# siyarvurucu/gym-macm

Measured on AMD Instinct MI355X. Metric: agent·steps/sec, cm-flock-v0 64 agents × 4096 envs, at 1/2/4/8 MI355X, higher is better.
Workload: dtype f32; 1 GPU; cm-flock-v0 n_agents=[64] x 4096 envs per GPU, uniform random discrete actions (MultiDiscrete[3,3,3]) pre-generated on device, from reset (seed 0x6d61636d); envs_per_gpu=4096, n_agents=64, total_envs=4096, split=weak: 4096 envs per GPU, parallelism=env-sharded x1 (no data-path collective), obs=float32, max_contacts=2016, spill_slots=4096, launch=one macm_world_rollout_traj launch for the K timed steps, outputs=every step's ([K, E, N, ...] trajectory buffers)

## Files before the change

### gym-macm_amd/csrc/flock_step_w64.hip

```cpp
#include "bots.hpp"
#include "flock_common.hpp"
#include "flock_spill.hpp"
#include "tdm_obs.hpp"

namespace macm {

constexpr int W = 64;
constexpr int TCAP = 256;
constexpr int DEG = 16;
constexpr int ICAP = W / 2;
constexpr int RCH = 2;
constexpr int KREC = 4;
constexpr int KRECA = KREC;
constexpr int kLevelsMinIsland = 4;
constexpr int kPrio2T = 3;

#if defined(MACM_STAMPS) && !defined(MACM_TIMELINE)
#define STAMP(k)                                                                    \
  do {                                                                              \
    __builtin_amdgcn_s_waitcnt(0);                                                  \
    const unsigned long long _t = __builtin_amdgcn_s_memtime();                     \
    if (lane == 0) B.stamps[(size_t)e * 16 + (k)] = _t;                             \
  } while (0)
#define STAMP_STAT(k, v)                                                            \
// ... 495 lines not shown
    win[2 * (K % kNearAhead)] = s_pc2[K + kNearAhead];
    win[2 * (K % kNearAhead) + 1] = s_pc2[16 + K + kNearAhead];
  }
  near2_min<2 * K, 32 + 2 * K, SCAL>(qa.x, qa.y, qb.x, qb.y, cme, st);
  near2_min<2 * K + 1, 33 + 2 * K, SCAL>(qa.z, qa.w, qb.z, qb.w, cme, st);
  if constexpr ((K & 1) == 1) __builtin_amdgcn_sched_barrier(0);
  if constexpr (K + 1 < 16) near2_step<K + 1, SCAL>(s_pc2, win, cme, st);
}

__device__ __forceinline__ unsigned long long moved_pairs(unsigned long long movedm, float4 fn, int lane) {
  unsigned long long row = 0ull;
  for (unsigned long long m = movedm; m; m &= m - 1ull) {
    const int j = __builtin_ctzll(m);
    const float jx = bcast(fn.x, j), jy = bcast(fn.y, j), jz = bcast(fn.z, j), jw = bcast(fn.w, j);
    const float sepv = fmaxf(fmaxf(jx - fn.z, jy - fn.w), fmaxf(fn.x - jz, fn.y - jw));
    const bool ov = !(0.0f < sepv);
    const unsigned long long colj = __ballot(ov);
    row |= (ov ? (1ull << j) : 0ull) | (lane == j ? colj : 0ull);
  }
  return row;
}

__device__ __forceinline__ int write_new_pairs(int lane, unsigned long long newmask, uint32_t* ocab,
                                               float2* ocimp, int C) {
  const int cnt = __popcll(newmask);
  const int pre = wave_prefix_sum(cnt);
  const int total = __builtin_amdgcn_readlane(pre, W - 1);
  int w = total - pre;
  unsigned long long m = newmask;
  while (m) {
    const int j = 63 - __clzll(m);
    m &= ~(1ull << j);
    if (w < C) {
      st_g<kState>(ocab + w, (uint32_t)lane | ((uint32_t)j << 16));
      st_g<kState>(ocimp + w, make_float2(0.0f, 0.0f));
    }
    ++w;
  }
  return total;
}

struct TailObs {
  unsigned long long* ctl;
  unsigned int tag;
  int nsteps;
  int k;
  bool worker;
  bool more;
  int q, left;
  int r, r_end;
  int nq;
};
constexpr int kTailChunk = 2;
constexpr unsigned kTailSpins = 1u << 20;

__device__ __forceinline__ unsigned long long* tail_counter(const TailObs& tl, int q) {
  return tl.ctl + (size_t)(((tl.tag & 1u) * kTailQ + q) * kTailLine);
}
// ... 56 lines not shown
    tl.more = false;
    return;
  }
  const size_t srow = ((size_t)k * E + e) * N;
  float4 sn = make_float4(0.0f, 0.0f, 0.0f, 0.0f);
  if (lane < N) sn = ld_wt4(TB.snap_out + srow + lane);
  const size_t row = ((size_t)(tl.k + k) * E + e) * N;
  s_c[lane] = make_float2(sn.x, sn.y);
  s_ang[lane] = sn.z;
  const unsigned long long livem = __ballot(lane < N && sn.w != 0.0f);
  __syncthreads();
  const size_t slots = row * (N - 1);
  OT* const obs_r = obs ? obs + slots * 4 : nullptr;
  uint8_t* const mask_r = TB.mask_out ? TB.mask_out + slots : nullptr;
  if constexpr (sizeof(OT) == 4) {
    if (staged) tdm_obs_rowblocks<OT>(obs_r, mask_r, N, lane, livem, TP, s_c, s_ang, stage, true);
    else tdm_obs_pairs<OT>(obs_r, mask_r, N, lane, livem, TP, s_c, s_ang);
  } else {
    tdm_obs_pairs<OT>(obs_r, mask_r, N, lane, livem, TP, s_c, s_ang);
  }
  __syncthreads();
}

template <int MODE, int NCAP, typename OT, bool SCAL = false>
__device__ __attribute__((always_inline)) inline void step_w64_body(
    const StepParams& P, const WorldBuffers& B, const TdmParams& TP, const TdmBuffers& TB, int cur,
    const void* __restrict__ actions, OT* __restrict__ obs, int32_t* __restrict__ nbr_out,
    float* __restrict__ rew_out, uint8_t* __restrict__ coll_out, uint8_t* __restrict__ done_out,
    const int e = blockIdx.x, const int lane = threadIdx.x, TailObs* tl = nullptr) {
  constexpr bool kT = MODE == kTdm;
#ifdef MACM_TIMELINE
  const unsigned long long tl_rt0 = __builtin_amdgcn_s_memrealtime(), tl_c0 = __builtin_amdgcn_s_memtime();
#endif
  const int N = P.n_agents;
  const int C = P.max_contacts;
  bool act = lane < N;
  const size_t ag = (size_t)e * N + lane;
  const int nxt = cur ^ 1;
  const unsigned long long lt = lanemask_lt(lane);

  __shared__ float2 s_c[W];
  __shared__ float2 s_v[W];
  constexpr int TMW = kT ? 1 : 2;
  struct __align__(32) Pool {
    float tn[2 * TCAP];
    uint32_t tab[TCAP];
    float tln[TCAP], tlt[TCAP];
    uint32_t tm[2 * TMW * W];
    uint32_t oldm[2 * W];
  };
  __shared__ Pool s_pool;
  static_assert(spill::layout(W, !kT).total <= (int)sizeof(Pool), "the spill step must fit the pool");
  uint32_t* const s_tab = s_pool.tab;
// ... 15 lines not shown
  __shared__ uint32_t s_cvis[TCAP / 32];
  __shared__ uint8_t s_deg[W], s_stack[W], s_ibodies[W], s_bisl[W];
  __shared__ uint16_t s_ic[ICAP + 1];
  __shared__ uint8_t s_ib[ICAP + 1];
  __shared__ uint8_t s_isolved[ICAP];
  __shared__ uint32_t s_imin[ICAP];
  __shared__ int s_nisl;
  __shared__ double s_hpd[W];
  __shared__ int8_t s_hit[W];
  __shared__ float s_ang[W];
#ifdef MACM_STAMPS
  __shared__ int s_stat_maxisl;
#endif
  if constexpr (kT) {
    if (tl && tl->worker) {
      tdm_tail_row<OT>(P, B, TP, TB, obs, *tl, lane, s_c, s_ang, reinterpret_cast<float4*>(&s_pool),
                       tdm_obs_rb_stage_bytes(N) <= (int)sizeof(Pool));
      return;
    }
  }

  const uint32_t* cab = B.cab[cur] + (size_t)e * C;
  const float2* cimp = B.cimp[cur] + (size_t)e * C;
  const int step_count = B.step_count[e];
  const int M = B.ccount[cur][e];
  float2 p = make_float2(0.0f, 0.0f), v = make_float2(0.0f, 0.0f), tg = make_float2(0.0f, 0.0f);
  float ang = 0.0f, slp = 0.0f;
  float4 fo = make_float4(0.0f, 0.0f, 0.0f, 0.0f);
  int a0 = 1, a1 = 1, a2 = 1, a3 = 0;
  float ax = 0.0f, ay = 0.0f;
  double hp = 0.0, cda = 0.0, cdm = 0.0;
  if (act) {
    p = B.pos[ag];
    v = B.vel[ag];
    ang = B.angle[ag];
    fo = B.fat[ag];
    slp = B.sleep[ag];
    if constexpr (kT) {
      const uchar4 a = reinterpret_cast<const uchar4*>(actions)[ag];
      a0 = a.x;
      a1 = a.y;
      a2 = a.z;
      a3 = a.w;
      act = TB.alive[ag] != 0;
      hp = TB.health[ag];
      cda = TB.cd_atk[ag];
      cdm = TB.cd_mov[ag];
    } else if (P.action_mode == MACM_ACTION_DISCRETE) {
      const uint8_t* a = (const uint8_t*)actions + ag * 3;
      a0 = a[0];
      a1 = a[1];
      a2 = a[2];
    } else {
      const float2 c = ((const float2*)actions)[ag];
      ax = c.x;
      ay = c.y;
    }
    if constexpr (!kT) tg = B.targets[(size_t)e * P.n_targets + B.tidx[lane]];
  }
  const bool act0 = act;
  double time_passed = 0.0;
  int st_prev = 0;
  unsigned long long ctr[4] = {0ull, 0ull, 0ull, 0ull};
  int2 lis = make_int2(0, -1);
  int win_prev = -1;
  uint8_t done_prev = 0;
  if (lane == 0) {
    time_passed = B.time_passed[e];
    st_prev = B.status[e];
    if constexpr (kT) {
      lis = TB.listener[e];
      win_prev = TB.winner[e];
      done_prev = B.done[e];
    }
    const ulonglong2* ec = reinterpret_cast<const ulonglong2*>(B.env_counters + (size_t)e * 4);
    const ulonglong2 c01 = ec[0], c23 = ec[1];
    ctr[0] = c01.x;
    ctr[1] = c01.y;
    ctr[2] = c23.x;
    ctr[3] = c23.y;
  }
  uint32_t rab[RCH];
  float2 rim[RCH];
#pragma unroll
  for (int c = 0; c < RCH; ++c) {
    const int k = c * W + lane;
    rab[c] = 0u;
    rim[c] = make_float2(0.0f, 0.0f);
    if (k < M) {
      rab[c] = cab[k];
      rim[c] = cimp[k];
    }
  }
  s_c[lane] = p;
  if (lane < TCAP / 32) s_cvis[lane] = 0u;
  s_oldm[2 * lane] = 0u;
#pragma unroll
  for (int q = 0; q < 2 * TMW; ++q) s_tm[2 * TMW * lane + q] = 0u;
  s_oldm[2 * lane + 1] = 0u;
  int status = 0;
  STAMP(0);

  float Fx = 0.0f, Fy = 0.0f;
  bool attacking = false;
  float ray_x = 0.0f, ray_y = 0.0f;
  if (act) {
    if (P.action_mode == MACM_ACTION_DISCRETE) {
      float af = (float)((double)ang + ((double)(a2 - 1) * P.rot_step) * P.inv_hz);
      double ad = (double)af;
      if (fabs(ad) > M_PI) {
        af = (float)(ad - sgn(ad) * (2.0 * M_PI));
        ad = (double)af;
      }
      ang = af;
// ... 147 lines not shown
  STAMP(2);

  const bool fast_dfs = T <= 64 * TMW;
  int deg = 0;
  unsigned long long tmask = 0ull, tmask1 = 0ull;
  if (fast_dfs) {
    if (act) {
      const uint32_t* tm = s_tm + 2 * TMW * lane;
      tmask = (unsigned long long)tm[0] | ((unsigned long long)tm[1] << 32);
      if (TMW == 2 && T > 64) tmask1 = (unsigned long long)tm[2] | ((unsigned long long)tm[3] << 32);
      deg = __popcll(tmask) + __popcll(tmask1);
    }
  } else if (act) {
    for (int t = 0; t < T; ++t) {
      const uint32_t ab = s_tab[t];
      if ((int)(ab & 0xffffu) == lane || (int)(ab >> 16) == lane) {
        if (deg < DEG) s_adj[lane * DEG + deg] = (uint8_t)t;
        ++deg;
      }
    }
  }
  if constexpr (!kT) {
    if (touch_over || (!fast_dfs && __builtin_amdgcn_ballot_w64(deg > DEG) != 0ull) || P.force_spill) {
      spill::step_env<OT, true>(P, B, e, cur, actions, obs, nbr_out, rew_out, coll_out, done_out,
                                reinterpret_cast<unsigned char*>(&s_pool));
      return;
    }
  } else {
    if (touch_over || (!fast_dfs && __builtin_amdgcn_ballot_w64(deg > DEG) != 0ull) || P.force_spill) {
      __shared__ int s_slot;
      const int slot = spill::acquire_slot(B, e, &s_slot);
      if (slot < 0) {
        spill::keep_lists(P, B, e, cur);
        if (lane == 0) {
          B.status[e] |= MACM_ST_SPILL_WAIT;
          report_status(B, MACM_ST_SPILL_WAIT);
        }
        return;
      }
      if (lane < N) {
        if (act0) {
          B.angle[ag] = ang;
          TB.cd_atk[ag] = cda;
          TB.cd_mov[ag] = cdm;
        }
        TB.health[ag] = hp;
// ... 2 lines not shown
        if (TB.alive_out) TB.alive_out[ag] = act ? 1 : 0;
      }
      if (lane == 0) {
        TB.listener[e] = lis;
        ulonglong2* ec = reinterpret_cast<ulonglong2*>(B.env_counters + (size_t)e * 4);
        ec[0] = make_ulonglong2(ctr[0] + (unsigned long long)__popcll(alive0_m),
                                ctr[1] + (unsigned long long)__popcll(att_m));
        B.env_counters[(size_t)e * 4 + 2] = ctr[2] + (unsigned long long)__popcll(alive0_m & ~livem);
      }
      const float2 F1 = make_float2(Fx, Fy);
      spill::step_env<OT, false, kTdm>(P, B, e, cur, actions, obs, nullptr, nullptr, nullptr, done_out,
                                        reinterpret_cast<unsigned char*>(&s_pool), &TP, &TB, &F1, slot);
      return;
    }
  }
  if (!fast_dfs && deg > DEG) {
    status |= MACM_ST_DEGREE_OVERFLOW;
    deg = DEG;
  }
  if (!fast_dfs) s_deg[lane] = (uint8_t)deg;
  const unsigned long long hasdeg = __ballot(act && deg > 0);
  __syncthreads();
  STAMP(3);
  if (hasdeg) __builtin_amdgcn_s_setprio(3);

  uint32_t ordv = 0u, lvlv = 0u, kislv = 0u;
  bool lvl_path = fast_dfs && T <= 64;
  if (fast_dfs) {
    const uint32_t tabv = lane < T ? s_tab[lane] : 0u;
    const uint32_t tabv1 = (TMW == 2 && 64 + lane < T) ? s_tab[64 + lane] : 0u;
    const uint32_t tm_lo = (uint32_t)tmask, tm_hi = (uint32_t)(tmask >> 32);
    const uint32_t tm1_lo = (uint32_t)tmask1, tm1_hi = (uint32_t)(tmask1 >> 32);
    uint32_t ordv1 = 0u, bodv = 0u, islv = 0u, icv = 0u, ibv = 0u, stk = 0u;
    int nord = 0, nisl = 0, nb = 0;
    auto dfs = [&](auto wide) {
    constexpr bool W2 = decltype(wide)::value;
    unsigned long long vis = ~hasdeg, cvis = 0ull, cvis1 = 0ull;
    for (unsigned long long todo = hasdeg; todo; todo = hasdeg & ~vis) {
      const int s = 63 - __clzll(todo);
      icv = writelane_m0(nord, nisl, icv);
      ibv = writelane_m0(nb, nisl, ibv);
      vis |= 1ull << s;
      stk = writelane_m0(s, 0, stk);
      int sp = 1;
      while (sp > 0) {
        --sp;
// ... 563 lines not shown
      near2_step<0, SCAL>(s_pc2, win, mk2(cx, cy), s2);
      const bool upper = s2.best_b < s2.best_a;
      best = upper ? s2.best_b : s2.best_a;
      bj = upper ? s2.bj_b : s2.bj_a;
    } else {
      NearState s1;
      s1.best = best;
      s1.bj = bj;
      float4 win[kNearAhead];
#pragma unroll
      for (int k = 0; k < kNearAhead; ++k) win[k] = s_pc2[k];
      near_step<0, NCAP>(s_pc2, win, mk2(cx, cy), s1);
      best = s1.best;
      bj = s1.bj;
    }
  }
  const unsigned long long myov = moved_pairs(movedm, fn, lane) & valid & ~(1ull << lane);
  const unsigned long long oldm = (unsigned long long)s_oldm[2 * lane] | ((unsigned long long)s_oldm[2 * lane + 1] << 32);
  const bool coll = act && ((myov | oldm) != 0ull);
  const unsigned long long above = lane == 63 ? 0ull : (~0ull << (lane + 1));
  const unsigned long long newmask = act ? (myov & ~oldm & above) : 0ull;
  STAMP(10);

  uint32_t* ocab = B.cab[nxt] + (size_t)e * C;
  float2* ocimp = B.cimp[nxt] + (size_t)e * C;
  const int nnew = write_new_pairs(lane, newmask, ocab, ocimp, C);
  int kept = 0, Tr = 0;
  for (int c = 0; c * W < M; ++c) {
    const int k = c * W + lane;
    uint32_t ab = 0u;
    if (c < RCH) {
#pragma unroll
      for (int q = 0; q < RCH; ++q)
        if (q == c) ab = rab[q];
    } else if (k < M) {
      ab = cab[k];
    }
    bool keep = false;
    const bool touch = (tbits >> c) & 1u;
    if (k < M) {
      const int a = ab & 0xffffu, b = ab >> 16;
      keep = overlap(s_fn[a], s_fn[b]);
    }
    const unsigned long long mt = __ballot(touch), mk = __ballot(keep);
    const int trank = Tr + __popcll(mt & lt);
    const int krank = kept + __popcll(mk & lt);
    Tr += __popcll(mt);
    kept += __popcll(mk);
    if (keep) {
      const int w = nnew + krank;
      if (w < C) {
        float2 l = make_float2(0.0f, 0.0f);
        if (touch && trank < TCAP) l = make_float2(s_tln[trank], s_tlt[trank]);
        st_g<kState>(ocab + w, ab);
        st_g<kState>(ocimp + w, l);
      }
    }
  }
  int total = nnew + kept;
  if (total > C) {
    status |= MACM_ST_CONTACT_OVERFLOW;
    total = C;
  }
  STAMP(11);

  float rew = 0.0f;
  if constexpr (!kT) {
    if (act) {
      const float tdx = tg.x - cx, tdy = tg.y - cy;
      const float td2 = tdx * tdx + tdy * tdy;
      const double d = sqrt((double)td2);
      if (coll) rew = -1.0f;
      else if (P.reward_mode == MACM_REWARD_LINEAR) rew = (float)((-d / 35) + 1);
      else rew = (d < P.reward_radius) ? 1.0f : 0.0f;
      st_g<kOut>(rew_out + ag, rew);
      if (coll_out) st_g<kOut>(coll_out + ag, (uint8_t)(coll ? 1 : 0));
      if (nbr_out) st_g<kOut>(nbr_out + ag, (int32_t)bj);
      if (obs) {
// ... 79 lines not shown
      }
      if (alive_teams == 0) dn = 1;
      TB.winner[e] = win;
      if (TB.winner_out) TB.winner_out[e] = win;
      TB.listener[e] = lis;
    }
    B.time_passed[e] = tp;
    B.done[e] = dn;
    if (done_out) done_out[e] = dn;
    B.step_count[e] = step_count + 1;
    B.ccount[nxt][e] = total;
    const int st = (mst1 ? 1 : 0) | (mst2 ? 2 : 0) | (mst4 ? 4 : 0);
    if (st) {
      B.status[e] = st_prev | st;
      report_status(B, st);
    }
    const unsigned long long c0 = kT ? (unsigned long long)__popcll(alive0_m) : (unsigned long long)N;
    ulonglong2* ec = reinterpret_cast<ulonglong2*>(B.env_counters + (size_t)e * 4);
    ec[0] = make_ulonglong2(ctr[0] + c0, ctr[1] + c1);
    ec[1] = make_ulonglong2(ctr[2] + c2, ctr[3] + (unsigned long long)dn);
    if constexpr (!kT) {
      if (P.reward_mode == MACM_REWARD_LINEAR) add_reward_sum(B, e, rsum);
    }
  }
  STAMP(13);
#ifdef MACM_TIMELINE
  {
    const unsigned long long rt1 = __builtin_amdgcn_s_memrealtime(), c1t = __builtin_amdgcn_s_memtime();
    const unsigned long long hw = (unsigned)__builtin_amdgcn_s_getreg((31 << 11) | 4);
    const unsigned long long xcc = (unsigned)__builtin_amdgcn_s_getreg((31 << 11) | 20);
    if (lane == 0) {
      unsigned long long* st = B.stamps + (size_t)e * 16;
      st[0] = tl_rt0;
      st[1] = tl_c0;
      st[2] = hw | (xcc << 32);
      st[3] = rt1;
      st[4] = c1t;
    }
  }
#endif
  STAMP_STAT(14, (unsigned long long)T | ((unsigned long long)nisl << 16) | ((unsigned long long)M << 32));
#ifdef MACM_STAMPS
  STAMP_STAT(15, (unsigned long long)s_stat_maxisl | ((unsigned long long)total << 32));
#endif
}

// ... 1 lines not shown

template <typename OT>
struct RolloutArgs {
  StepParams P;
  WorldBuffers B;
  TdmParams TP;
  TdmBuffers TB;
  const void* actions;
  OT* obs;
  int32_t* nbr_out;
  float* rew_out;
  uint8_t* coll_out;
  uint8_t* done_out;
  unsigned long long astride;
  int cur;
  int nsteps;
  uint8_t* policy_act;
  int traj;
  int sched_off;
  unsigned long long* tail_ctl;
  unsigned int tail_tag;
  int tail_k0;
};

template <typename T>
__device__ __forceinline__ T* traj_row(T* p, size_t k, size_t per_step) {
  return p ? p + k * per_step : p;
}

constexpr int kRollBalanceMinSteps = 32;
constexpr int kSchedMaxSize = 4095;

__global__ __launch_bounds__(1024) void rollout_sched(const uint32_t* __restrict__ ccount, uint32_t* __restrict__ order,
                                                     int E, int C, unsigned int* reset2 = nullptr) {
  extern __shared__ uint32_t s_h[];
  __shared__ int s_scan[32];
  const int tid = threadIdx.x, BS = blockDim.x;
  if (reset2 && tid < 2) reset2[tid] = 0u;
  for (int i = tid; i <= C; i += BS) s_h[i] = 0u;
  __syncthreads();
  for (int e = tid; e < E; e += BS) atomicAdd(&s_h[max(0, min((int)ccount[e], C))], 1u);
  __syncthreads();
  {
    const int per = (C + 1 + BS - 1) / BS, hi = C - tid * per, lo = max(-1, hi - per);
    int sum = 0;
    for (int c = hi; c > lo; --c) sum += (int)s_h[c];
    int run;
    spill::block_scan_excl(sum, run, s_scan);
    for (int c = hi; c > lo; --c) {
      const int n = (int)s_h[c];
      s_h[c] = (uint32_t)run;
      run += n;
    }
  }
  __syncthreads();
  for (int e = tid; e < E; e += BS) order[atomicAdd(&s_h[max(0, min((int)ccount[e], C))], 1u)] = (uint32_t)e;
}

template <int MODE, int NCAP, typename OT, bool SCAL = false>
__global__ __launch_bounds__(W) __attribute__((amdgpu_waves_per_eu(4))) void env_rollout_w64(RolloutArgs<OT> A0) {
  const int nsteps = A0.nsteps;
  const bool bal = A0.B.sched && nsteps >= kRollBalanceMinSteps;
  const bool phys = MODE != kTdm || (int)blockIdx.x < A0.P.n_envs;
  const int env = bal && phys ? (int)A0.B.sched[A0.sched_off + blockIdx.x] : (int)blockIdx.x;
  const int nq = gridDim.x < (unsigned)kTailQ ? (int)gridDim.x : kTailQ;
  TailObs tl{};
  tl.ctl = A0.tail_tag ? A0.tail_ctl : nullptr;
  tl.tag = A0.tail_tag;
  tl.nsteps = nsteps - A0.tail_k0;
  tl.k = 0;
  tl.worker = false;
  tl.more = true;
  tl.q = (int)(blockIdx.x % nq);
  tl.left = 1;
  tl.r = 0;
  tl.r_end = 0;
  tl.nq = nq;
  const int ksteps = phys ? nsteps : 0;
  for (int k = 0; k < ksteps; ++k) {
    const __attribute__((address_space(4))) RolloutArgs<OT>* ka =
        (const __attribute__((address_space(4))) RolloutArgs<OT>*)__builtin_amdgcn_kernarg_segment_ptr();
    asm volatile("" : "+s"(ka));
    const RolloutArgs<OT>& A = *(const RolloutArgs<OT>*)ka;
    const int N = A.P.n_agents, lane = threadIdx.x;
    const size_t EN = (size_t)A.P.n_envs * N;
    const size_t kr = A.traj ? (size_t)k : 0;
    const size_t od = MODE == kTdm ? (size_t)(N - 1) * 4 : (A.P.coord == MACM_COORD_CARTESIAN ? 6 : 4);
    OT* const obs = traj_row(A.obs, kr, EN * od);
    TdmBuffers TB = A.TB;
    if constexpr (MODE == kTdm) {
      TB.mask_out = traj_row(TB.mask_out, kr, EN * (N - 1));
      TB.health_out = traj_row(TB.health_out, kr, EN);
      TB.alive_out = traj_row(TB.alive_out, kr, EN);
      TB.winner_out = traj_row(TB.winner_out, kr, (size_t)A.P.n_envs);
      TB.snap_out = A.tail_tag ? (k >= A.tail_k0 ? traj_row(TB.snap_out, (size_t)(k - A.tail_k0), EN) : nullptr)
                               : traj_row(TB.snap_out, kr, EN);
    }
    const size_t abytes = MODE == kTdm ? 4 : 3;
    uint8_t* const pol_in = A.policy_act ? A.policy_act + kr * EN * abytes : nullptr;
    __builtin_amdgcn_s_setprio(0);
    int sl = (int)threadIdx.x;
    if constexpr (MODE == kTdm) asm volatile("" : "+v"(sl));
    tl.k = k - A0.tail_k0;
    step_w64_body<MODE, NCAP, OT, SCAL>(A.P, A.B, A.TP, TB, A.cur ^ (k & 1),
                                        pol_in ? pol_in : static_cast<const unsigned char*>(A.actions) + (size_t)k * A.astride,
                                        obs, traj_row(A.nbr_out, kr, EN), traj_row(A.rew_out, kr, EN),
                                        traj_row(A.coll_out, kr, EN), traj_row(A.done_out, kr, (size_t)A.P.n_envs),
                                        env, sl, MODE == kTdm ? &tl : nullptr);
    __builtin_amdgcn_fence(__ATOMIC_SEQ_CST, "workgroup");
    __syncthreads();
    if (pol_in) {
      uint8_t* const pol_out = A.traj ? pol_in + EN * abytes : pol_in;
      if (lane < N) {
        const size_t row = (size_t)env * N + lane;
        if constexpr (MODE == kTdm)
          bot_combat_row(obs + row * (N - 1) * 4, TB.mask_out + row * (N - 1), N, pol_out + row * 4);
        else
          bot_flock_row(obs + row * od, (int)od, pol_out + row * 3);
      }
      __builtin_amdgcn_fence(__ATOMIC_SEQ_CST, "workgroup");
      __syncthreads();
    }
  }
  if constexpr (MODE == kTdm) {
    if (tl.ctl) {
      if (phys) {
        __builtin_amdgcn_s_waitcnt(0);
        if (threadIdx.x == 0)
          __hip_atomic_store(tl.ctl + 2 * kTailQ * kTailLine + env, ((unsigned long long)tl.tag << 32) | (unsigned)tl.nsteps,
                             __ATOMIC_RELAXED, __HIP_MEMORY_SCOPE_AGENT);
      }
      if (blockIdx.x == 0 && threadIdx.x < kTailQ)
        __hip_atomic_store(tl.ctl + (size_t)((((tl.tag + 1u) & 1u) * kTailQ + threadIdx.x) * kTailLine), 0ull,
                           __ATOMIC_RELAXED, __HIP_MEMORY_SCOPE_AGENT);
      tl.worker = true;
      tl.k = A0.tail_k0;
      int sl = (int)threadIdx.x;
      asm volatile("" : "+v"(sl));
      while (tl.more)
        step_w64_body<MODE, NCAP, OT, SCAL>(A0.P, A0.B, A0.TP, A0.TB, A0.cur, nullptr, A0.obs, nullptr, nullptr, nullptr,
                                            nullptr, env, sl, &tl);
    }
  }
}

int tdm_rollout_resident_blocks(int n_agents, bool obs_f64) {
  const void* k = n_agents <= 32 ? (obs_f64 ? (const void*)env_rollout_w64<kTdm, 32, double>
                                            : (const void*)env_rollout_w64<kTdm, 32, float>)
                                 : (obs_f64 ? (const void*)env_rollout_w64<kTdm, 64, double>
                                            : (const void*)env_rollout_w64<kTdm, 64, float>);
  int per = 0, dev = 0, cus = 0;
  if (hipOccupancyMaxActiveBlocksPerMultiprocessor(&per, k, W, 0) != hipSuccess || hipGetDevice(&dev) != hipSuccess ||
      hipDeviceGetAttribute(&cus, hipDeviceAttributeMultiprocessorCount, dev) != hipSuccess) {
    (void)hipGetLastError();
    return 0;
  }
  return per * cus;
}

template <int MODE, int NCAP, typename OT, bool SCAL = false>
static void launch_roll(int nsteps, unsigned long long astride, int traj, hipStream_t s, const StepParams& P,
                        const WorldBuffers& B, const TdmParams& TP, const TdmBuffers& TB, int cur, const void* actions,
                        void* obs, int32_t* nbr, float* rew, uint8_t* coll, uint8_t* done,
                        unsigned long long* tail_ctl = nullptr, unsigned tail_tag = 0u, int tail_workers = 0,
                        int tail_k0 = 0) {
  uint8_t* pol = astride == 0 ? static_cast<uint8_t*>(const_cast<void*>(actions)) : nullptr;
  const bool bal = B.sched && nsteps >= kRollBalanceMinSteps;
  if (bal) {
    const int CB = P.max_contacts < kSchedMaxSize ? P.max_contacts : kSchedMaxSize;
    hipLaunchKernelGGL(rollout_sched, dim3(1), dim3(1024), sizeof(uint32_t) * (CB + 1), s,
                       reinterpret_cast<const uint32_t*>(B.ccount[cur]), B.sched, P.n_envs, CB, nullptr);
    if (hipPeekAtLastError() != hipSuccess) return;
  }
  RolloutArgs<OT> A{P, B, TP, TB, actions, (OT*)obs, nbr, rew, coll, done, astride, cur, nsteps, pol, traj, 0,
                    tail_ctl, tail_tag, tail_tag ? tail_k0 : 0};
  const int blocks = P.n_envs + (tail_tag ? tail_workers : 0);
  hipLaunchKernelGGL((env_rollout_w64<MODE, NCAP, OT, SCAL>), dim3(blocks), dim3(W), 0, s, A);
}

hipError_t launch_env_order(const uint32_t* ccount, uint32_t* order, int E, int C, hipStream_t s, unsigned int* reset2) {
  const int CB = C < kSchedMaxSize ? C : kSchedMaxSize;
  hipLaunchKernelGGL(rollout_sched, dim3(1), dim3(1024), sizeof(uint32_t) * (CB + 1), s, ccount, order, E, CB, reset2);
  return hipGetLastError();
}

hipError_t launch_rollout_w64(const StepParams& P, const WorldBuffers& B, int cur, const void* actions, void* obs,
                              bool obs_f64, int32_t* nbr, float* rew, uint8_t* coll, uint8_t* done, hipStream_t s,
                              int nsteps, unsigned long long astride, int traj) {
  const TdmParams TP{};
  const TdmBuffers TB{};
  const bool small = P.n_agents <= 32;
  if (obs_f64) {
    if (small)
      launch_roll<kFlock, 32, double>(nsteps, astride, traj, s, P, B, TP, TB, cur, actions, obs, nbr, rew, coll, done);
    else
      launch_roll<kFlock, 64, double>(nsteps, astride, traj, s, P, B, TP, TB, cur, actions, obs, nbr, rew, coll, done);
  } else {
    if (small)
      launch_roll<kFlock, 32, float>(nsteps, astride, traj, s, P, B, TP, TB, cur, actions, obs, nbr, rew, coll, done);
    else if (P.n_envs >= kScalarSweepMinEnvs)
      launch_roll<kFlock, 64, float, true>(nsteps, astride, traj, s, P, B, TP, TB, cur, actions, obs, nbr, rew, coll,
                                           done);
    else
      launch_roll<kFlock, 64, float>(nsteps, astride, traj, s, P, B, TP, TB, cur, actions, obs, nbr, rew, coll, done);
  }
  return hipGetLastError();
}

hipError_t launch_tdm_rollout_w64(const StepParams& P, const WorldBuffers& B, const TdmParams& TP,
                                  const TdmBuffers& TB, int cur, const void* actions, void* obs, bool obs_f64,
                                  uint8_t* done, hipStream_t s, int nsteps, unsigned long long astride, int traj,
                                  unsigned long long* tail_ctl, unsigned tail_tag, int tail_workers,
                                  int tail_k0) {
  const bool small = P.n_agents <= 32;
  if (obs_f64) {
    if (small)
      launch_roll<kTdm, 32, double>(nsteps, astride, traj, s, P, B, TP, TB, cur, actions, obs, nullptr, nullptr,
                                    nullptr, done, tail_ctl, tail_tag, tail_workers, tail_k0);
    else
      launch_roll<kTdm, 64, double>(nsteps, astride, traj, s, P, B, TP, TB, cur, actions, obs, nullptr, nullptr,
                                    nullptr, done, tail_ctl, tail_tag, tail_workers, tail_k0);
  } else {
    if (small)
      launch_roll<kTdm, 32, float>(nsteps, astride, traj, s, P, B, TP, TB, cur, actions, obs, nullptr, nullptr,
                                   nullptr, done, tail_ctl, tail_tag, tail_workers, tail_k0);
    else
      launch_roll<kTdm, 64, float>(nsteps, astride, traj, s, P, B, TP, TB, cur, actions, obs, nullptr, nullptr,
// ... 291 lines not shown
```

### gym-macm_amd/csrc/macm_capi.hip

```cpp
#include <math.h>
#include <stdio.h>
#include <string.h>

#include <algorithm>
#include <string>
#include <vector>

#include "flock_common.hpp"
#include "py_mt19937.hpp"

namespace macm {
hipError_t launch_step_w64(const StepParams& P, const WorldBuffers& B, int cur, const void* actions, void* obs,
                           bool obs_f64, int32_t* nbr, float* rew, uint8_t* coll, uint8_t* done, hipStream_t s);
hipError_t launch_rollout_w64(const StepParams& P, const WorldBuffers& B, int cur, const void* actions, void* obs,
                              bool obs_f64, int32_t* nbr, float* rew, uint8_t* coll, uint8_t* done, hipStream_t s,
                              int nsteps, unsigned long long astride, int traj);
hipError_t launch_init_w64(const StepParams& P, const WorldBuffers& B, int cur, void* obs, bool obs_f64,
                           int32_t* nbr, const uint8_t* mask, hipStream_t s);
hipError_t launch_observe_w64(const StepParams& P, const WorldBuffers& B, void* obs, bool obs_f64, int32_t* nbr,
                              hipStream_t s);
hipError_t launch_step_wg(const StepParams& P, const WorldBuffers& B, int cur, int tcap, const void* actions,
                          void* obs, bool obs_f64, int32_t* nbr, float* rew, uint8_t* coll, uint8_t* done,
                          hipStream_t s, HandoffStream* HS, uint8_t* bot_act = nullptr);
hipError_t launch_init_wg(const StepParams& P, const WorldBuffers& B, int cur, void* obs, bool obs_f64, int32_t* nbr,
                          const uint8_t* mask, hipStream_t s);
hipError_t launch_observe_wg(const StepParams& P, const WorldBuffers& B, void* obs, bool obs_f64, int32_t* nbr,
                             hipStream_t s);
hipError_t launch_tdm_step_w64(const StepParams& P, const WorldBuffers& B, const TdmParams& TP,
                               const TdmBuffers& TB, int cur, const void* actions, void* obs, bool obs_f64,
                               uint8_t* done, hipStream_t s);
hipError_t launch_tdm_rollout_w64(const StepParams& P, const WorldBuffers& B, const TdmParams& TP,
                                  const TdmBuffers& TB, int cur, const void* actions, void* obs, bool obs_f64,
                                  uint8_t* done, hipStream_t s, int nsteps, unsigned long long astride, int traj,
                                  unsigned long long* tail_ctl = nullptr, unsigned tail_tag = 0u, int tail_workers = 0,
                                  int tail_k0 = 0);
int tdm_rollout_resident_blocks(int n_agents, bool obs_f64);
hipError_t launch_tdm_init_w64(const StepParams& P, const WorldBuffers& B, const TdmParams& TP,
                               const TdmBuffers& TB, int cur, void* obs, bool obs_f64, const uint8_t* mask,
                               hipStream_t s);
// ... 37 lines not shown

struct macm_world {
  macm_config cfg;
  StepParams P;
  WorldBuffers B;
  int cur;
  int device;
  bool wave;
  bool big;
  int tcap;
  std::vector<int32_t> tidx;
  std::vector<void*> allocs;
  uint32_t* mt = nullptr;
  uint8_t* rmask = nullptr;
  bool mt_valid = false;
  uint32_t* hstat = nullptr;
  unsigned long long* bad = nullptr;
  std::vector<hipStream_t> slice_streams;
  std::vector<hipEvent_t> slice_events;
  HandoffStream* ho = nullptr;
  bool ho_tried = false;
  int slots_alloc = 0;
  int pool0 = 0;
};

struct macm_tdm {
  macm_tdm_config cfg;
  StepParams P;
  WorldBuffers B;
  TdmParams TP;
  TdmBuffers TB;
  int cur;
  int device;
  bool wave;
  std::vector<int> team;
  std::vector<void*> allocs;
  uint32_t* mt = nullptr;
  uint8_t* rmask = nullptr;
  bool mt_valid = false;
  uint32_t* hstat = nullptr;
  unsigned long long* bad = nullptr;
  int slots_alloc = 0;
  int pool0 = 0;
  float4* snap = nullptr;
  size_t snap_rows = 0;
  hipStream_t obs_stream = nullptr;
// ... 649 lines not shown

static int world_rollout(macm_world* w, const void* actions, int n_steps, const macm_outputs* out, void* stream,
                         bool bots, bool traj) {
  if (n_steps < 0) return fail(MACM_E_INVALID, "n_steps must be >= 0");
  if (n_steps == 0) return MACM_OK;
  if (!w || !actions || !out || !out->reward) return fail(MACM_E_INVALID, "world/actions/out/reward is NULL");
  if (bots && !out->obs) return fail(MACM_E_INVALID, "out->obs is NULL (the bots act on it)");
  if (bots && w->cfg.action_mode != MACM_ACTION_DISCRETE) return fail(MACM_E_INVALID, "bots.flock acts in discrete mode");
  if (const uint32_t st = read_host_status(w->hstat)) return overflow_error(st);
  DeviceGuard g(w->device);
  hipStream_t s = (hipStream_t)stream;
  const int mode = w->cfg.action_mode == MACM_ACTION_DISCRETE ? 0 : 1;
  if (w->cfg.validate_actions) {
    const long long rows = (long long)(bots ? 1 : n_steps) * w->P.n_envs;
    if (rows > INT32_MAX) return fail(MACM_E_INVALID, "n_steps * n_envs too large to validate");
    const int rc = check_actions(w->bad, actions, mode, nullptr, (int)rows, w->P.n_agents, s, w->P.n_envs);
    if (rc) return rc;
  }
  const unsigned long long astride =
      bots ? 0ull
           : (unsigned long long)w->P.n_envs * w->P.n_agents * (mode == 0 ? 3 * sizeof(uint8_t) : 2 * sizeof(float));
  if (w->wave) {
    HIP_TRY(launch_rollout_w64(w->P, w->B, w->cur, actions, out->obs, w->cfg.obs_f64 != 0, out->nbr_id, out->reward,
                               out->collided, out->done, s, n_steps, astride, traj ? 1 : 0));
    if (n_steps & 1) w->cur ^= 1;
    return MACM_OK;
  }
  const unsigned char* act = static_cast<const unsigned char*>(actions);
  if (const int S = wg_rollout_slices(w)) return rollout_wg_slices(w, S, act, n_steps, astride, out, traj, s);
  const long long rows = (long long)w->P.n_envs * w->P.n_agents;
  const unsigned long long kstride = bots ? (traj ? (unsigned long long)rows * 3 : 0ull) : astride;
  for (int k = 0; k < n_steps; ++k) {
    const macm_outputs ok = step_outputs(w, out, k, traj);
    const unsigned char* act_k = act + k * kstride;
    if (w->big)
      HIP_TRY(launch_step_big(w->P, w->B, w->cur, act_k, ok.obs, w->cfg.obs_f64 != 0, ok.nbr_id, ok.reward,
                              ok.collided, ok.done, s));
    else
      HIP_TRY(launch_step_wg(w->P, w->B, w->cur, w->tcap, act_k, ok.obs, w->cfg.obs_f64 != 0, ok.nbr_id, ok.reward,
                             ok.collided, ok.done, s, handoff_for(w),
                             bots ? const_cast<unsigned char*>(act_k) + (traj ? rows * 3 : 0) : nullptr));
    w->cur ^= 1;
    if (bots && w->big)
      HIP_TRY(launch_bots_flock(ok.obs, w->cfg.obs_f64 != 0, obs_dim(w->cfg), rows,
                                const_cast<unsigned char*>(act_k) + (traj ? rows * 3 : 0), s));
  }
  return MACM_OK;
// ... 206 lines not shown
extern "C++" template <typename Wt>
static int set_spill_pool(Wt* w, int32_t flags, int pool) {
  const bool want = (flags & MACM_DEBUG_SPILL_POOL) != 0;
  const bool never = (flags & MACM_DEBUG_SPILL_FAIL) != 0;
  if (want && never) return fail(MACM_E_INVALID, "SPILL_POOL and SPILL_FAIL exclude each other");
  if (want && (pool < 1 || pool > w->slots_alloc))
    return fail(MACM_E_INVALID, "SPILL_POOL: 1 <= slots <= the " + std::to_string(w->slots_alloc) + " allocated");
  const int target = never ? -1 : want ? pool : w->pool0;
  if (target == w->B.sp_pool) return MACM_OK;
  DeviceGuard g(w->device);
  HIP_TRY(hipDeviceSynchronize());
  if (target > 0) {
    if (!w->B.sp_lock && dalloc(w->allocs, &w->B.sp_lock, (size_t)w->slots_alloc)) return MACM_E_OOM;
    HIP_TRY(hipMemset(w->B.sp_lock, 0, sizeof(uint32_t) * w->slots_alloc));
  }
  w->B.sp_pool = target;
  return MACM_OK;
}

int macm_world_set_debug(macm_world* w, int32_t flags) {
  if (!w) return fail(MACM_E_INVALID, "world is NULL");
  const int pool = (flags & MACM_DEBUG_SPILL_POOL) ? (flags >> 8) : 0;
  flags &= 0xff;
  if (flags & ~(MACM_DEBUG_FORCE_SPILL | MACM_DEBUG_SWEEP_CELLS | MACM_DEBUG_SWEEP_ALL_PAIRS | MACM_DEBUG_SPILL_POOL | MACM_DEBUG_SPILL_FAIL))
    return fail(MACM_E_INVALID, "unknown debug flag");
  if ((flags & MACM_DEBUG_SWEEP_CELLS) && (flags & MACM_DEBUG_SWEEP_ALL_PAIRS))
    return fail(MACM_E_INVALID, "SWEEP_CELLS and SWEEP_ALL_PAIRS exclude each other");
  if (int rc = set_spill_pool(w, flags, pool)) return rc;
  w->P.force_spill = (flags & MACM_DEBUG_FORCE_SPILL) ? 1 : 0;
  w->P.sweep = (flags & MACM_DEBUG_SWEEP_CELLS) ? 1 : (flags & MACM_DEBUG_SWEEP_ALL_PAIRS) ? 2 : 0;
  return MACM_OK;
}


int macm_tdm_config_default(macm_tdm_config* c) {
  if (!c) return fail(MACM_E_INVALID, "cfg is NULL");
  memset(c, 0, sizeof(*c));
  c->n_teams = 2;
  c->team_size[0] = 1;
  c->team_size[1] = 1;
  c->n_agents = 2;
  c->velocity_iterations = 8;
  c->position_iterations = 3;
  c->warm_starting = 1;
  c->obs_f64 = 0;
  c->fresh_raycast = 0;
  c->decay_mov_penalty = 0;
  c->hz = 60.0;
  c->world_width = 30.0;
  c->world_height = 30.0;
  c->agent_rotation_speed = 0.8 * (2 * M_PI);
  c->agent_force = 20.0;
// ... 696 lines not shown
```

### gym-macm_amd/gym_macm/_abi.py

```python
from __future__ import annotations

import ctypes
import os
from ctypes import (POINTER, Structure, c_char_p, c_double, c_float, c_int, c_int32, c_int64,
                    c_uint8, c_uint64, c_void_p)

ACTION_DISCRETE, ACTION_CONTINUOUS = 0, 1
REWARD_BINARY, REWARD_LINEAR = 0, 1
COORD_POLAR, COORD_CARTESIAN = 0, 1

ST_CONTACT_OVERFLOW, ST_TOUCH_OVERFLOW, ST_DEGREE_OVERFLOW, ST_INVALID_ACTION, ST_SPILL_WAIT = 1, 2, 4, 8, 16
ST_HANDOFF = 32
DEBUG_FORCE_SPILL = 1
DEBUG_SWEEP_CELLS = 2
DEBUG_SWEEP_ALL_PAIRS = 4
DEBUG_SPILL_POOL = 8
DEBUG_SPILL_FAIL = 16
E_INVALID, E_OVERFLOW = -1, -5

_ERRORS = {
    -1: "MACM_E_INVALID",
    -2: "MACM_E_OOM",
    -3: "MACM_E_HIP",
    -4: "MACM_E_UNSUPPORTED",
    -5: "MACM_E_OVERFLOW",
}


class MacmConfig(Structure):
    _fields_ = [
        ("n_agents", c_int32),
        ("n_targets", c_int32),
        ("action_mode", c_int32),
        ("reward_mode", c_int32),
        ("coord", c_int32),
        ("velocity_iterations", c_int32),
        ("position_iterations", c_int32),
        ("warm_starting", c_int32),
        ("obs_f64", c_int32),
        ("validate_actions", c_int32),
# ... 227 lines not shown
```

### include/macm.h

```cpp
#ifndef MACM_H
#define MACM_H

#include <stdint.h>

#ifdef __cplusplus
extern "C" {
#endif

#define MACM_ABI_VERSION 9

enum {
  MACM_OK = 0,
  MACM_E_INVALID = -1,
  MACM_E_OOM = -2,
  MACM_E_HIP = -3,
  MACM_E_UNSUPPORTED = -4,
  MACM_E_OVERFLOW = -5
};

enum { MACM_ACTION_DISCRETE = 0, MACM_ACTION_CONTINUOUS = 1 };
enum { MACM_REWARD_BINARY = 0, MACM_REWARD_LINEAR = 1 };
enum { MACM_COORD_POLAR = 0, MACM_COORD_CARTESIAN = 1 };

enum {
  MACM_ST_CONTACT_OVERFLOW = 1,
  MACM_ST_TOUCH_OVERFLOW = 2,
  MACM_ST_DEGREE_OVERFLOW = 4,
  MACM_ST_INVALID_ACTION = 8,
  MACM_ST_SPILL_WAIT = 16,
  MACM_ST_HANDOFF = 32
};

enum {
  MACM_DEBUG_FORCE_SPILL = 1,
  MACM_DEBUG_SWEEP_CELLS = 2,
  MACM_DEBUG_SWEEP_ALL_PAIRS = 4,
  MACM_DEBUG_SPILL_POOL = 8,
  MACM_DEBUG_SPILL_FAIL = 16
};

typedef struct macm_config {
  int32_t n_agents;
  int32_t n_targets;
  int32_t action_mode;
  int32_t reward_mode;
  int32_t coord;
  int32_t velocity_iterations;
  int32_t position_iterations;
  int32_t warm_starting;
  int32_t obs_f64;
  int32_t validate_actions;
  double hz;
  double start_spread;
  double start_point[2];
  double agent_rotation_speed;
  double agent_force;
  double time_limit;
  double reward_radius;
  double target_mindist;
  double target_maxdist;
  float radius;
// ... 200 lines not shown
```

Before: 22.02 billion agent·steps/s.

## Carry per-agent state and contacts in registers across rollout steps

In the Flock rollout kernel with supplied actions, each step now keeps per-agent position, velocity, angle, fatigue, sleep, target, step count, the next step's actions and up to RCH*W contact pairs and impulses in a register/LDS carry struct. The next step reads these instead of reloading them from global memory, and contacts are staged in shared memory as they are written. The aim is to cut global loads and the load latency at the start of every step. The carry is invalidated when contacts overflow, on a spill, on other status flags, or when a debug reload flag is set. The cost is more register pressure, extra LDS writes, and a more complex control path that may hurt occupancy.

```diff
diff --git a/gym-macm_amd/csrc/flock_step_w64.hip b/gym-macm_amd/csrc/flock_step_w64.hip
--- a/gym-macm_amd/csrc/flock_step_w64.hip
+++ b/gym-macm_amd/csrc/flock_step_w64.hip
@@ -541,7 +541,8 @@
 }
 
 __device__ __forceinline__ int write_new_pairs(int lane, unsigned long long newmask, uint32_t* ocab,
-                                               float2* ocimp, int C) {
+                                               float2* ocimp, int C, uint32_t* stage_ab = nullptr,
+                                               float2* stage_im = nullptr) {
   const int cnt = __popcll(newmask);
   const int pre = wave_prefix_sum(cnt);
   const int total = __builtin_amdgcn_readlane(pre, W - 1);
@@ -553,6 +554,10 @@
     if (w < C) {
       st_g<kState>(ocab + w, (uint32_t)lane | ((uint32_t)j << 16));
       st_g<kState>(ocimp + w, make_float2(0.0f, 0.0f));
+      if (stage_ab && w < RCH * W) {
+        stage_ab[w] = (uint32_t)lane | ((uint32_t)j << 16);
+        stage_im[w] = make_float2(0.0f, 0.0f);
+      }
     }
     ++w;
   }
@@ -655,13 +660,26 @@
   __syncthreads();
 }
 
-template <int MODE, int NCAP, typename OT, bool SCAL = false>
+struct StepCarry {
+  bool valid;
+  float2 p, v, tg;
+  float ang, slp;
+  float4 fat;
+  uint32_t rab[RCH];
+  float2 rim[RCH];
+  uint32_t ar0, ar1;
+  int M, step_count;
+};
+
+template <int MODE, int NCAP, typename OT, bool SCAL = false, bool CARRY = false>
 __device__ __attribute__((always_inline)) inline void step_w64_body(
     const StepParams& P, const WorldBuffers& B, const TdmParams& TP, const TdmBuffers& TB, int cur,
     const void* __restrict__ actions, OT* __restrict__ obs, int32_t* __restrict__ nbr_out,
     float* __restrict__ rew_out, uint8_t* __restrict__ coll_out, uint8_t* __restrict__ done_out,
-    const int e = blockIdx.x, const int lane = threadIdx.x, TailObs* tl = nullptr) {
+    const int e = blockIdx.x, const int lane = threadIdx.x, TailObs* tl = nullptr, StepCarry* carry = nullptr,
+    const void* actions_next = nullptr) {
   constexpr bool kT = MODE == kTdm;
+  static_assert(!CARRY || !kT, "the carried step is Flock's");
 #ifdef MACM_TIMELINE
   const unsigned long long tl_rt0 = __builtin_amdgcn_s_memrealtime(), tl_c0 = __builtin_amdgcn_s_memtime();
 #endif
@@ -723,15 +741,20 @@
 
   const uint32_t* cab = B.cab[cur] + (size_t)e * C;
   const float2* cimp = B.cimp[cur] + (size_t)e * C;
-  const int step_count = B.step_count[e];
-  const int M = B.ccount[cur][e];
+  bool carried = false;
+  if constexpr (CARRY) carried = carry->valid;
+  int step_count = 0, M = 0;
+  if (!carried) {
+    step_count = B.step_count[e];
+    M = B.ccount[cur][e];
+  }
   float2 p = make_float2(0.0f, 0.0f), v = make_float2(0.0f, 0.0f), tg = make_float2(0.0f, 0.0f);
   float ang = 0.0f, slp = 0.0f;
   float4 fo = make_float4(0.0f, 0.0f, 0.0f, 0.0f);
   int a0 = 1, a1 = 1, a2 = 1, a3 = 0;
   float ax = 0.0f, ay = 0.0f;
   double hp = 0.0, cda = 0.0, cdm = 0.0;
-  if (act) {
+  if (act && !carried) {
     p = B.pos[ag];
     v = B.vel[ag];
     ang = B.angle[ag];
@@ -766,7 +789,7 @@
   int2 lis = make_int2(0, -1);
   int win_prev = -1;
   uint8_t done_prev = 0;
-  if (lane == 0) {
+  if (lane == 0 && !CARRY) {
     time_passed = B.time_passed[e];
     st_prev = B.status[e];
     if constexpr (kT) {
@@ -791,6 +814,28 @@
     if (k < M) {
       rab[c] = cab[k];
       rim[c] = cimp[k];
+    }
+  }
+  if constexpr (CARRY) {
+    if (carried) {
+      step_count = carry->step_count;
+      M = carry->M;
+      p = carry->p;
+      v = carry->v;
+      tg = carry->tg;
+      ang = carry->ang;
+      slp = carry->slp;
+      fo = carry->fat;
+      a0 = (int)(carry->ar0 & 0xffu);
+      a1 = (int)(carry->ar0 >> 8);
+      a2 = (int)carry->ar1;
+      ax = __uint_as_float(carry->ar0);
+      ay = __uint_as_float(carry->ar1);
+#pragma unroll
+      for (int c = 0; c < RCH; ++c) {
+        rab[c] = carry->rab[c];
+        rim[c] = carry->rim[c];
+      }
     }
   }
   s_c[lane] = p;
@@ -984,6 +1029,10 @@
   }
   if constexpr (!kT) {
     if (touch_over || (!fast_dfs && __builtin_amdgcn_ballot_w64(deg > DEG) != 0ull) || P.force_spill) {
+      if constexpr (CARRY) {
+        if (carried) __builtin_amdgcn_fence(__ATOMIC_SEQ_CST, "workgroup");
+        carry->valid = false;
+      }
       spill::step_env<OT, true>(P, B, e, cur, actions, obs, nbr_out, rew_out, coll_out, done_out,
                                 reinterpret_cast<unsigned char*>(&s_pool));
       return;
@@ -1032,6 +1081,22 @@
   const unsigned long long hasdeg = __ballot(act && deg > 0);
   __syncthreads();
   STAMP(3);
+  if constexpr (CARRY) {
+    const bool discrete = P.action_mode == MACM_ACTION_DISCRETE;
+    carry->ar0 = discrete ? 0x0101u : 0u;
+    carry->ar1 = discrete ? 1u : 0u;
+    if (actions_next && act) {
+      if (discrete) {
+        const uint8_t* a = (const uint8_t*)actions_next + ag * 3;
+        carry->ar0 = (uint32_t)a[0] | ((uint32_t)a[1] << 8);
+        carry->ar1 = a[2];
+      } else {
+        const uint2 c = ((const uint2*)actions_next)[ag];
+        carry->ar0 = c.x;
+        carry->ar1 = c.y;
+      }
+    }
+  }
   if (hasdeg) __builtin_amdgcn_s_setprio(3);
 
   uint32_t ordv = 0u, lvlv = 0u, kislv = 0u;
@@ -1641,9 +1706,25 @@
   const unsigned long long newmask = act ? (myov & ~oldm & above) : 0ull;
   STAMP(10);
 
+  if constexpr (CARRY) {
+    if (lane == 0) {
+      time_passed = B.time_passed[e];
+      st_prev = B.status[e];
+      const ulonglong2* ec = reinterpret_cast<const ulonglong2*>(B.env_counters + (size_t)e * 4);
+      const ulonglong2 c01 = ec[0], c23 = ec[1];
+      ctr[0] = c01.x;
+      ctr[1] = c01.y;
+      ctr[2] = c23.x;
+      ctr[3] = c23.y;
+    }
+  }
   uint32_t* ocab = B.cab[nxt] + (size_t)e * C;
   float2* ocimp = B.cimp[nxt] + (size_t)e * C;
-  const int nnew = write_new_pairs(lane, newmask, ocab, ocimp, C);
+  uint32_t* const stage_ab = CARRY ? s_tab : nullptr;
+  float2* const stage_im = CARRY ? reinterpret_cast<float2*>(s_tm) : nullptr;
+  static_assert(sizeof(uint32_t) * RCH * W <= sizeof(s_pool.tab), "the staged entries must fit in s_tab");
+  static_assert(!CARRY || sizeof(float2) * RCH * W <= sizeof(s_pool.tm), "the staged impulses must fit in s_tm");
+  const int nnew = write_new_pairs(lane, newmask, ocab, ocimp, C, stage_ab, stage_im);
   int kept = 0, Tr = 0;
   for (int c = 0; c * W < M; ++c) {
     const int k = c * W + lane;
@@ -1673,6 +1754,12 @@
         if (touch && trank < TCAP) l = make_float2(s_tln[trank], s_tlt[trank]);
         st_g<kState>(ocab + w, ab);
         st_g<kState>(ocimp + w, l);
+        if constexpr (CARRY) {
+          if (w < RCH * W) {
+            stage_ab[w] = ab;
+            stage_im[w] = l;
+          }
+        }
       }
     }
   }
@@ -1798,6 +1885,28 @@
     if constexpr (!kT) {
       if (P.reward_mode == MACM_REWARD_LINEAR) add_reward_sum(B, e, rsum);
     }
+  }
+  if constexpr (CARRY) {
+    carry->p = make_float2(cx, cy);
+    carry->v = make_float2(vx, vy);
+    carry->ang = ang;
+    carry->fat = fn;
+    carry->slp = ns;
+    carry->tg = tg;
+    carry->M = total;
+    carry->step_count = step_count + 1;
+    __syncthreads();
+#pragma unroll
+    for (int c = 0; c < RCH; ++c) {
+      const int k = c * W + lane;
+      carry->rab[c] = 0u;
+      carry->rim[c] = make_float2(0.0f, 0.0f);
+      if (k < total) {
+        carry->rab[c] = stage_ab[k];
+        carry->rim[c] = stage_im[k];
+      }
+    }
+    carry->valid = total <= RCH * W && !(mst1 | mst2 | mst4);
   }
   STAMP(13);
 #ifdef MACM_TIMELINE
@@ -1845,6 +1954,7 @@
   unsigned int tail_tag;
   int tail_k0;
 };
+constexpr int kRollReloadBit = 2;
 
 template <typename T>
 __device__ __forceinline__ T* traj_row(T* p, size_t k, size_t per_step) {
@@ -1880,7 +1990,7 @@
   for (int e = tid; e < E; e += BS) order[atomicAdd(&s_h[max(0, min((int)ccount[e], C))], 1u)] = (uint32_t)e;
 }
 
-template <int MODE, int NCAP, typename OT, bool SCAL = false>
+template <int MODE, int NCAP, typename OT, bool SCAL = false, bool CARRY = false>
 __global__ __launch_bounds__(W) __attribute__((amdgpu_waves_per_eu(4))) void env_rollout_w64(RolloutArgs<OT> A0) {
   const int nsteps = A0.nsteps;
   const bool bal = A0.B.sched && nsteps >= kRollBalanceMinSteps;
@@ -1900,6 +2010,7 @@
   tl.r_end = 0;
   tl.nq = nq;
   const int ksteps = phys ? nsteps : 0;
+  StepCarry cy{};
   for (int k = 0; k < ksteps; ++k) {
     const __attribute__((address_space(4))) RolloutArgs<OT>* ka =
         (const __attribute__((address_space(4))) RolloutArgs<OT>*)__builtin_amdgcn_kernarg_segment_ptr();
@@ -1925,24 +2036,35 @@
     int sl = (int)threadIdx.x;
     if constexpr (MODE == kTdm) asm volatile("" : "+v"(sl));
     tl.k = k - A0.tail_k0;
-    step_w64_body<MODE, NCAP, OT, SCAL>(A.P, A.B, A.TP, TB, A.cur ^ (k & 1),
-                                        pol_in ? pol_in : static_cast<const unsigned char*>(A.actions) + (size_t)k * A.astride,
-                                        obs, traj_row(A.nbr_out, kr, EN), traj_row(A.rew_out, kr, EN),
-                                        traj_row(A.coll_out, kr, EN), traj_row(A.done_out, kr, (size_t)A.P.n_envs),
-                                        env, sl, MODE == kTdm ? &tl : nullptr);
-    __builtin_amdgcn_fence(__ATOMIC_SEQ_CST, "workgroup");
-    __syncthreads();
-    if (pol_in) {
-      uint8_t* const pol_out = A.traj ? pol_in + EN * abytes : pol_in;
-      if (lane < N) {
-        const size_t row = (size_t)env * N + lane;
-        if constexpr (MODE == kTdm)
-          bot_combat_row(obs + row * (N - 1) * 4, TB.mask_out + row * (N - 1), N, pol_out + row * 4);
-        else
-          bot_flock_row(obs + row * od, (int)od, pol_out + row * 3);
-      }
+    if constexpr (CARRY) {
+      const unsigned char* const act_k = static_cast<const unsigned char*>(A.actions) + (size_t)k * A.astride;
+      step_w64_body<MODE, NCAP, OT, SCAL, true>(A.P, A.B, A.TP, TB, (A.cur ^ k) & 1, act_k, obs,
+                                                traj_row(A.nbr_out, kr, EN), traj_row(A.rew_out, kr, EN),
+                                                traj_row(A.coll_out, kr, EN), traj_row(A.done_out, kr, (size_t)A.P.n_envs),
+                                                env, sl, nullptr, &cy, k + 1 < ksteps ? act_k + A.astride : nullptr);
+      if (A.cur & kRollReloadBit) cy.valid = false;
+      if (!cy.valid) __builtin_amdgcn_fence(__ATOMIC_SEQ_CST, "workgroup");
+      __syncthreads();
+    } else {
+      step_w64_body<MODE, NCAP, OT, SCAL>(A.P, A.B, A.TP, TB, A.cur ^ (k & 1),
+                                          pol_in ? pol_in : static_cast<const unsigned char*>(A.actions) + (size_t)k * A.astride,
+                                          obs, traj_row(A.nbr_out, kr, EN), traj_row(A.rew_out, kr, EN),
+                                          traj_row(A.coll_out, kr, EN), traj_row(A.done_out, kr, (size_t)A.P.n_envs),
+                                          env, sl, MODE == kTdm ? &tl : nullptr);
       __builtin_amdgcn_fence(__ATOMIC_SEQ_CST, "workgroup");
       __syncthreads();
+      if (pol_in) {
+        uint8_t* const pol_out = A.traj ? pol_in + EN * abytes : pol_in;
+        if (lane < N) {
+          const size_t row = (size_t)env * N + lane;
+          if constexpr (MODE == kTdm)
+            bot_combat_row(obs + row * (N - 1) * 4, TB.mask_out + row * (N - 1), N, pol_out + row * 4);
+          else
+            bot_flock_row(obs + row * od, (int)od, pol_out + row * 3);
+        }
+        __builtin_amdgcn_fence(__ATOMIC_SEQ_CST, "workgroup");
+        __syncthreads();
+      }
     }
   }
   if constexpr (MODE == kTdm) {
@@ -1986,7 +2108,7 @@
                         const WorldBuffers& B, const TdmParams& TP, const TdmBuffers& TB, int cur, const void* actions,
                         void* obs, int32_t* nbr, float* rew, uint8_t* coll, uint8_t* done,
                         unsigned long long* tail_ctl = nullptr, unsigned tail_tag = 0u, int tail_workers = 0,
-                        int tail_k0 = 0) {
+                        int tail_k0 = 0, int reload = 0) {
   uint8_t* pol = astride == 0 ? static_cast<uint8_t*>(const_cast<void*>(actions)) : nullptr;
   const bool bal = B.sched && nsteps >= kRollBalanceMinSteps;
   if (bal) {
@@ -1998,6 +2120,13 @@
   RolloutArgs<OT> A{P, B, TP, TB, actions, (OT*)obs, nbr, rew, coll, done, astride, cur, nsteps, pol, traj, 0,
                     tail_ctl, tail_tag, tail_tag ? tail_k0 : 0};
   const int blocks = P.n_envs + (tail_tag ? tail_workers : 0);
+  if constexpr (MODE == kFlock) {
+    if (!pol) {
+      if (reload) A.cur |= kRollReloadBit;
+      hipLaunchKernelGGL((env_rollout_w64<MODE, NCAP, OT, SCAL, true>), dim3(blocks), dim3(W), 0, s, A);
+      return;
+    }
+  }
   hipLaunchKernelGGL((env_rollout_w64<MODE, NCAP, OT, SCAL>), dim3(blocks), dim3(W), 0, s, A);
 }
 
@@ -2009,23 +2138,27 @@
 
 hipError_t launch_rollout_w64(const StepParams& P, const WorldBuffers& B, int cur, const void* actions, void* obs,
                               bool obs_f64, int32_t* nbr, float* rew, uint8_t* coll, uint8_t* done, hipStream_t s,
-                              int nsteps, unsigned long long astride, int traj) {
+                              int nsteps, unsigned long long astride, int traj, int reload) {
   const TdmParams TP{};
   const TdmBuffers TB{};
   const bool small = P.n_agents <= 32;
   if (obs_f64) {
     if (small)
-      launch_roll<kFlock, 32, double>(nsteps, astride, traj, s, P, B, TP, TB, cur, actions, obs, nbr, rew, coll, done);
+      launch_roll<kFlock, 32, double>(nsteps, astride, traj, s, P, B, TP, TB, cur, actions, obs, nbr, rew, coll, done,
+                                     nullptr, 0u, 0, 0, reload);
     else
-      launch_roll<kFlock, 64, double>(nsteps, astride, traj, s, P, B, TP, TB, cur, actions, obs, nbr, rew, coll, done);
+      launch_roll<kFlock, 64, double>(nsteps, astride, traj, s, P, B, TP, TB, cur, actions, obs, nbr, rew, coll, done,
+                                     nullptr, 0u, 0, 0, reload);
   } else {
     if (small)
-      launch_roll<kFlock, 32, float>(nsteps, astride, traj, s, P, B, TP, TB, cur, actions, obs, nbr, rew, coll, done);
+      launch_roll<kFlock, 32, float>(nsteps, astride, traj, s, P, B, TP, TB, cur, actions, obs, nbr, rew, coll, done,
+                                     nullptr, 0u, 0, 0, reload);
     else if (P.n_envs >= kScalarSweepMinEnvs)
       launch_roll<kFlock, 64, float, true>(nsteps, astride, traj, s, P, B, TP, TB, cur, actions, obs, nbr, rew, coll,
-                                           done);
+                                           done, nullptr, 0u, 0, 0, reload);
     else
-      launch_roll<kFlock, 64, float>(nsteps, astride, traj, s, P, B, TP, TB, cur, actions, obs, nbr, rew, coll, done);
+      launch_roll<kFlock, 64, float>(nsteps, astride, traj, s, P, B, TP, TB, cur, actions, obs, nbr, rew, coll, done,
+                                     nullptr, 0u, 0, 0, reload);
   }
   return hipGetLastError();
 }
diff --git a/gym-macm_amd/csrc/macm_capi.hip b/gym-macm_amd/csrc/macm_capi.hip
--- a/gym-macm_amd/csrc/macm_capi.hip
+++ b/gym-macm_amd/csrc/macm_capi.hip
@@ -14,7 +14,7 @@
                            bool obs_f64, int32_t* nbr, float* rew, uint8_t* coll, uint8_t* done, hipStream_t s);
 hipError_t launch_rollout_w64(const StepParams& P, const WorldBuffers& B, int cur, const void* actions, void* obs,
                               bool obs_f64, int32_t* nbr, float* rew, uint8_t* coll, uint8_t* done, hipStream_t s,
-                              int nsteps, unsigned long long astride, int traj);
+                              int nsteps, unsigned long long astride, int traj, int reload);
 hipError_t launch_init_w64(const StepParams& P, const WorldBuffers& B, int cur, void* obs, bool obs_f64,
                            int32_t* nbr, const uint8_t* mask, hipStream_t s);
 hipError_t launch_observe_w64(const StepParams& P, const WorldBuffers& B, void* obs, bool obs_f64, int32_t* nbr,
@@ -98,6 +98,7 @@
   bool ho_tried = false;
   int slots_alloc = 0;
   int pool0 = 0;
+  int roll_reload = 0;
 };
 
 struct macm_tdm {
@@ -793,7 +794,7 @@
            : (unsigned long long)w->P.n_envs * w->P.n_agents * (mode == 0 ? 3 * sizeof(uint8_t) : 2 * sizeof(float));
   if (w->wave) {
     HIP_TRY(launch_rollout_w64(w->P, w->B, w->cur, actions, out->obs, w->cfg.obs_f64 != 0, out->nbr_id, out->reward,
-                               out->collided, out->done, s, n_steps, astride, traj ? 1 : 0));
+                               out->collided, out->done, s, n_steps, astride, traj ? 1 : 0, w->roll_reload));
     if (n_steps & 1) w->cur ^= 1;
     return MACM_OK;
   }
@@ -1046,12 +1047,14 @@
   if (!w) return fail(MACM_E_INVALID, "world is NULL");
   const int pool = (flags & MACM_DEBUG_SPILL_POOL) ? (flags >> 8) : 0;
   flags &= 0xff;
-  if (flags & ~(MACM_DEBUG_FORCE_SPILL | MACM_DEBUG_SWEEP_CELLS | MACM_DEBUG_SWEEP_ALL_PAIRS | MACM_DEBUG_SPILL_POOL | MACM_DEBUG_SPILL_FAIL))
+  if (flags & ~(MACM_DEBUG_FORCE_SPILL | MACM_DEBUG_SWEEP_CELLS | MACM_DEBUG_SWEEP_ALL_PAIRS | MACM_DEBUG_SPILL_POOL | MACM_DEBUG_SPILL_FAIL |
+                MACM_DEBUG_ROLLOUT_RELOAD))
     return fail(MACM_E_INVALID, "unknown debug flag");
   if ((flags & MACM_DEBUG_SWEEP_CELLS) && (flags & MACM_DEBUG_SWEEP_ALL_PAIRS))
     return fail(MACM_E_INVALID, "SWEEP_CELLS and SWEEP_ALL_PAIRS exclude each other");
   if (int rc = set_spill_pool(w, flags, pool)) return rc;
   w->P.force_spill = (flags & MACM_DEBUG_FORCE_SPILL) ? 1 : 0;
+  w->roll_reload = (flags & MACM_DEBUG_ROLLOUT_RELOAD) ? 1 : 0;
   w->P.sweep = (flags & MACM_DEBUG_SWEEP_CELLS) ? 1 : (flags & MACM_DEBUG_SWEEP_ALL_PAIRS) ? 2 : 0;
   return MACM_OK;
 }
diff --git a/gym-macm_amd/gym_macm/_abi.py b/gym-macm_amd/gym_macm/_abi.py
--- a/gym-macm_amd/gym_macm/_abi.py
+++ b/gym-macm_amd/gym_macm/_abi.py
@@ -16,6 +16,7 @@
 DEBUG_SWEEP_ALL_PAIRS = 4
 DEBUG_SPILL_POOL = 8
 DEBUG_SPILL_FAIL = 16
+DEBUG_ROLLOUT_RELOAD = 32
 E_INVALID, E_OVERFLOW = -1, -5
 
 _ERRORS = {
diff --git a/include/macm.h b/include/macm.h
--- a/include/macm.h
+++ b/include/macm.h
@@ -36,7 +36,8 @@
   MACM_DEBUG_SWEEP_CELLS = 2,
   MACM_DEBUG_SWEEP_ALL_PAIRS = 4,
   MACM_DEBUG_SPILL_POOL = 8,
-  MACM_DEBUG_SPILL_FAIL = 16
+  MACM_DEBUG_SPILL_FAIL = 16,
+  MACM_DEBUG_ROLLOUT_RELOAD = 32
 };
 
 typedef struct macm_config {
```

After: 22.74 billion agent·steps/s (median of 6 runs). 3.2% higher.
